# aluo-x/3D_SLN

Measured on AMD Instinct MI355X. Metric: scene-graph VAE steps/sec + 256² diff-render fps, 1/2/4/8 MI355X, higher is better.
Workload: dtype f32; 1 GPU; BASELINE configs[1]: batch=64 scene graphs x (32 objects, 64 triples) per GPU, Sg2ScVAE train step at train.py defaults (embedding_dim=64, 5+5 GraphTripleConv, BatchNorm); O=2048, T=4096, hipgraph=True, distinct_batches_cycled=4, eps=N(0,1) drawn on the device inside the step, parallelism=dp1

## Files before the change

3d_sln_amd/_lib.py:

```python
from __future__ import annotations

import ctypes as C
import os

HERE = os.path.dirname(os.path.abspath(__file__))
LIB_PATH = os.path.join(HERE, "libsln_hip.so")

SLN_E = {-1: "SLN_E_BADARG", -2: "SLN_E_UNSUPPORTED", -3: "SLN_E_STATE", -4: "SLN_E_NOGPU", -5: "SLN_E_NOMEM", -6: "SLN_E_CAPTURE"}

c_f32p = C.c_void_p
c_i64p = C.c_void_p


class SlnError(RuntimeError):
    pass


class SlnVaeConfig(C.Structure):
    _fields_ = [(n, C.c_int) for n in (
        "embedding_dim", "gconv_num_layers", "recurrent", "batch_norm", "decoder_cat", "use_ae",
        "box_dim", "n_angle", "num_objs", "num_preds", "num_attrs", "no_attr")]


class SlnVaeUnit(C.Structure):
# ... 200 lines not shown
                                    C.c_void_p, C.c_int, C.c_int, C.c_int, C.c_void_p, C.c_int64, c_f32p, c_f32p, C.c_void_p]),
    "sln_gconv_net_create": (C.c_int, [C.c_int, C.c_int, C.c_int, C.c_int, C.c_int, C.c_int, C.POINTER(C.c_void_p)]),
    "sln_gconv_net_set_edges": (C.c_int, [C.c_void_p, C.c_void_p, C.c_int, C.c_int, C.c_void_p]),
    "sln_gconv_net_forward": (C.c_int, [C.c_void_p, c_f32p, c_f32p, c_f32p, c_f32p, C.c_int, C.c_void_p]),
    "sln_gconv_net_backward": (C.c_int, [C.c_void_p, c_f32p, c_f32p, c_f32p, c_f32p, C.c_void_p]),
    "sln_linear_forward": (C.c_int, [c_f32p, C.c_int, C.c_int, c_f32p, c_f32p, c_f32p, C.c_int, C.c_void_p,
                                     C.c_int, C.c_void_p]),
    "sln_linear_wgrad": (C.c_int, [c_f32p, c_f32p, C.c_int, C.c_int, C.c_int, c_f32p, c_f32p, C.c_void_p]),
    "sln_debug_gemm_nt": (C.c_int, [C.POINTER(SlnDbgGemmNT), C.c_int, C.POINTER(C.c_int), C.c_void_p]),
    "sln_debug_gemm_tn": (C.c_int, [C.POINTER(SlnDbgGemmTN), C.c_int, C.c_int, C.c_void_p]),
    "sln_debug_gemm_nt_route": (C.c_int, [C.POINTER(SlnDbgGemmNT), C.POINTER(SlnDbgNTRoute)]),
    "sln_debug_gemm_nt_half": (C.c_int, [C.POINTER(SlnDbgGemmNT), C.c_int, C.c_void_p]),
    "sln_debug_gemm_nt_half_takes": (C.c_int, [C.POINTER(SlnDbgGemmNT)]),
    "sln_debug_gemm_sizes": (C.c_int, [C.POINTER(C.c_int), C.c_int]),
    "sln_debug_vae_csr": (C.c_int, [c_i64p, C.c_int, C.c_int, C.c_int, C.POINTER(SlnDbgCsr), C.c_void_p, C.c_void_p]),
    "sln_debug_vae_edge": (C.c_int, [C.POINTER(SlnDbgEdge), C.c_int, C.c_int, C.POINTER(C.c_int), C.c_void_p]),
    "sln_debug_vae_loss": (C.c_int, [C.POINTER(SlnDbgLoss), C.c_void_p]),
    "sln_debug_vae_tables": (C.c_int, [C.c_int, C.c_void_p, C.c_int, C.c_int, C.c_float, C.c_int, C.c_int, C.c_int, C.c_void_p]),
    "sln_debug_vae_embed": (C.c_int, [C.POINTER(SlnDbgEmbed), C.c_int, C.c_int, C.POINTER(C.c_int), C.c_void_p]),
    "sln_debug_vae_opt": (C.c_int, [C.POINTER(SlnDbgOpt), C.c_void_p]),
    "sln_debug_vae_sizes": (C.c_int, [C.POINTER(C.c_int), C.c_int]),
    "sln_debug_vae_leaf_launches": (C.c_int64, [C.c_void_p]),
    "sln_debug_vae_half_launches": (C.c_int64, [C.c_void_p]),
    "sln_project_faces": (C.c_int, [c_f32p, C.c_void_p, c_f32p, c_f32p, c_f32p, C.c_int, C.c_int, C.c_int, C.c_float, C.c_float, c_f32p, C.c_void_p]),
    "sln_project_faces_backward": (C.c_int, [c_f32p, C.c_void_p, c_f32p, c_f32p, c_f32p, C.c_int, C.c_int, C.c_int, C.c_float, C.c_float, c_f32p,
                                             c_f32p, C.c_void_p]),
    "sln_raster_workspace_bytes": (C.c_int64, [C.c_int, C.c_int]),
    "sln_raster_forward": (C.c_int, [c_f32p, C.c_int, C.c_int, C.c_int, C.c_float, C.c_float, C.c_void_p, C.c_void_p,
                                     c_f32p, c_f32p, C.c_void_p]),
    "sln_raster_forward_dual": (C.c_int, [c_f32p, C.c_int, C.c_int, C.c_int, C.c_float, C.c_float, C.c_float, C.c_void_p,
                                          C.c_void_p, c_f32p, c_f32p, C.c_void_p, c_f32p, c_f32p, C.c_void_p]),
    "sln_raster_texture_sample": (C.c_int, [c_f32p, c_f32p, C.c_void_p, c_f32p, c_f32p, C.c_int, C.c_int, C.c_int, C.c_int,
                                            C.c_float, c_f32p, C.c_void_p]),
    "sln_raster_backward_depth": (C.c_int, [c_f32p, C.c_void_p, c_f32p, c_f32p, c_f32p, C.c_int, C.c_int, C.c_int, c_f32p,
                                            C.c_void_p]),
    "sln_raster_backward_rgb": (C.c_int, [c_f32p, C.c_void_p, c_f32p, c_f32p, C.c_int, C.c_int, C.c_int, C.c_int, C.c_float,
                                          c_f32p, C.c_void_p]),
    "sln_raster_texture_sample_chw": (C.c_int, [c_f32p, c_f32p, C.c_void_p, c_f32p, c_f32p, C.c_int, C.c_int, C.c_int, C.c_int, C.c_int,
                                                C.c_float, C.c_float, c_f32p, C.c_void_p]),
    "sln_raster_backward_rgb_multi": (C.c_int, [c_f32p, C.c_void_p, C.c_void_p, C.c_void_p, C.c_int, C.c_int, C.c_int, C.c_int, C.c_float,
                                                C.c_void_p, c_f32p, C.c_void_p]),
    "sln_scene_workspace_bytes": (C.c_int64, [C.c_int, C.c_int, C.c_int]),
    "sln_scene_forward": (C.c_int, [c_f32p, C.c_void_p, C.c_int, C.c_int, C.c_int, C.c_int, C.c_void_p, C.c_void_p,
                                    C.c_float, C.c_float, C.c_float, C.c_float, C.c_void_p, c_f32p, C.c_void_p]),
    "sln_scene_forward_live": (C.c_int, [c_f32p, C.c_void_p, C.c_int, C.c_int, C.c_int, C.c_int, C.c_void_p, C.c_void_p,
                                         C.c_float, C.c_float, C.c_float, C.c_float, C.c_void_p, c_f32p, C.c_void_p, C.c_void_p, C.c_void_p]),
# ... 150 lines not shown
```

3d_sln_amd/csrc/gemm_f32.hip:

```cpp
#include <cstdio>
#include <cstdlib>
#include <algorithm>
#include <vector>
#include "gemm_bodies.h"
#include "vae_multi.h"
namespace {
constexpr bool nt_coef_helpers(int amode, int epi) { return amode != 2 || epi == EPI_MASK; }
template <int BM, int BN, int AMODE, int EPI>
constexpr bool nt_helpers() { return BM == 64 && BN == 64 && nt_coef_helpers(AMODE, EPI); }
template <int BM, int BN, int WM, int WN, int AMODE, int EPI, int MULTI>
__global__ __launch_bounds__((nt_helpers<BM, BN, AMODE, EPI>() ? 512 : 256)) void gemm_nt_kernel(const GemmNTArgs a) {
  extern __shared__ __attribute__((aligned(16))) char smem[];
  gemm_nt_body<BM, BN, WM, WN, AMODE, EPI, MULTI, nt_helpers<BM, BN, AMODE, EPI>()>(a, blockIdx.x, ((a.M + BM - 1) / BM) * ((a.N + BN - 1) / BN), smem);
}

template <int AMODE, int EPI>
constexpr bool nt_helpers2() { return nt_coef_helpers(AMODE, EPI); }
template <int J, int AMODE, int EPI>
__global__ __launch_bounds__((nt_helpers2<AMODE, EPI>() ? 512 : 256)) void gemm_nt16_kernel(const GemmNTArgs a) {
  extern __shared__ __attribute__((aligned(16))) char smem[];
  gemm_nt_body16<J, AMODE, EPI, nt_helpers2<AMODE, EPI>()>(a, blockIdx.x, ((a.M + 63) / 64) * ((a.N + 32 * J - 1) / (32 * J)), smem);
}

template <int AMODE, int EPI, int NSEG = 1>
// ... 264 lines not shown
#define SLN_NT64M(AM, EP, MU) if (am == AM && ep == EP && mu == MU) return launch_nt64_multi<AM, EP, MU>(tab, tiles_dev, R, max_tiles, smem64, st);
    SLN_NT64M(0, EPI_PLAIN, 0) SLN_NT64M(0, EPI_PLAIN, 1) SLN_NT64M(0, EPI_PLAIN, 2) SLN_NT64M(0, EPI_MASK, 0) SLN_NT64M(0, EPI_MASK, 1) SLN_NT64M(0, EPI_MASK, 2)
    SLN_NT64M(2, EPI_PLAIN, 0) SLN_NT64M(2, EPI_PLAIN, 1) SLN_NT64M(2, EPI_PLAIN, 2) SLN_NT64M(2, EPI_MASK, 0) SLN_NT64M(2, EPI_MASK, 1) SLN_NT64M(2, EPI_MASK, 2)
#undef SLN_NT64M
    return -1;
  }
  const size_t smem = nt_small_smem_bytes(max_K);
  const int amode = key / 16, epi = (key / 4) % 4, nseg = key % 4;
#define SLN_NTM(AM, EP, NS) if (amode == AM && epi == EP && nseg == NS) return launch_nt_small_multi<AM, EP, NS>(tab, tiles_dev, R, max_tiles, smem, st);
  SLN_NTM(0, EPI_PLAIN, 1) SLN_NTM(0, EPI_PLAIN, 3) SLN_NTM(0, EPI_MASK, 1) SLN_NTM(0, EPI_MASK, 3)
  SLN_NTM(2, EPI_PLAIN, 1) SLN_NTM(2, EPI_PLAIN, 3) SLN_NTM(2, EPI_MASK, 1) SLN_NTM(2, EPI_MASK, 3)
#undef SLN_NTM
  return -1;
}

int sln_launch_gemm_tn(const GemmTNArgs& a0, hipStream_t st) {
  SlnProfScope prof(SLN_FAM_GEMM_TN, 2.0 * a0.R * a0.Nout * a0.Kin, st);
  GemmTNArgs a = a0;
  const bool x2 = tn_prepare(a);
  if (x2) return launch_tn<64, 64, 2, 2, true>(a, st);
  return launch_tn<64, 64, 2, 2, false>(a, st);
}

int sln_tn_multi_plan(GemmTNArgs* probs, int n, TnMultiMeta* meta, int* blocks, bool* x2, bool* xg, double* flops) {
  if (n < 1 || n > SLN_TN_MULTI_MAX) return -1;
  static const int target0 = std::getenv("SLN_TN_MULTI_ROWS") ? std::atoi(std::getenv("SLN_TN_MULTI_ROWS")) : 768;
  static const bool no_xcd = std::getenv("SLN_TN_NO_XCD") != nullptr;
  bool any_x2 = false, any_xg = false;
  double work = 0.0;
  for (int i = 0; i < n; ++i) {
    const GemmTNArgs& a = probs[i];
    if (a.R <= 0 || a.Nout <= 0 || a.Kin <= 0 || !tn_supported(a)) return -1;
    for (int s = 0; s < a.G.nseg; ++s) any_x2 |= a.G.seg[s].x2 != nullptr;
    any_xg |= tn_gathers(a);
    work += 2.0 * a.R * a.Nout * a.Kin;
  }
  struct Group { int prob, chunk, tiles; long cost; };
  std::vector<Group> groups;
  int per_xcd[8];
  std::vector<int> owner;
  for (long target = g_sln_deterministic ? (1L << 30) : (target0 > 0 ? target0 : 1024);; target *= 2) {
    groups.clear();
    for (int i = 0; i < n; ++i) {
      GemmTNArgs& a = probs[i];
      const int chunks = sln_cdiv(a.R, (int)(target > a.R ? a.R : target));
      a.rows_per_block = sln_cdiv(sln_cdiv(a.R, chunks), BK) * BK;
      const int tiles = sln_cdiv(a.Nout, 64) * sln_cdiv(a.Kin, 64), nch = sln_cdiv(a.R, a.rows_per_block);
      for (int c = 0; c < nch; ++c) {
        const int rows = (c + 1) * a.rows_per_block <= a.R ? a.rows_per_block : a.R - c * a.rows_per_block;
        groups.push_back(Group{i, c, tiles, (long)tiles * rows});
      }
    }
    std::stable_sort(groups.begin(), groups.end(), [](const Group& x, const Group& y) { return x.cost > y.cost; });
    long load[8] = {0, 0, 0, 0, 0, 0, 0, 0};
    for (int x = 0; x < 8; ++x) per_xcd[x] = 0;
    owner.assign(groups.size(), 0);
    for (size_t g = 0; g < groups.size(); ++g) {
      int best = 0;
      if (no_xcd) best = (int)(g % 8);
      else for (int x = 1; x < 8; ++x) if (load[x] < load[best]) best = x;
      owner[g] = best; load[best] += groups[g].cost; per_xcd[best] += groups[g].tiles;
    }
    int mx = 0;
    for (int x = 0; x < 8; ++x) mx = per_xcd[x] > mx ? per_xcd[x] : mx;
    if (8 * mx <= SLN_TN_MULTI_ITEMS) break;
    if (target > (1L << 30)) return -1;
  }
  if (any_xg) {
    const int* any = nullptr;
    for (int i = 0; i < n; ++i) { if (probs[i].X.idx_a) any = probs[i].X.idx_a; else if (probs[i].X.idx_b) any = probs[i].X.idx_b; }
    for (int i = 0; i < n; ++i) if (!probs[i].X.idx_a && !probs[i].X.idx_b) probs[i].X.idx_a = any;
  }
  int mx = 0;
  for (int x = 0; x < 8; ++x) mx = per_xcd[x] > mx ? per_xcd[x] : mx;
  std::memset(meta, 0, sizeof(*meta));
  meta->nprob = n; meta->nblocks = 8 * mx;
  for (int b = 0; b < 8 * mx; ++b) meta->item[b].prob = -1;
  int fill[8] = {0, 0, 0, 0, 0, 0, 0, 0};
  for (size_t g = 0; g < groups.size(); ++g) {
    const int x = owner[g];
    for (int t = 0; t < groups[g].tiles; ++t) {
      TnMultiItem& it = meta->item[8 * (fill[x]++) + x];
      it.prob = groups[g].prob; it.tile = t; it.chunk = groups[g].chunk;
    }
  }
  *blocks = 8 * mx; *x2 = any_x2; *xg = any_xg; *flops = work;
  return 0;
}

int sln_launch_gemm_tn_multi(const GemmTNArgs* dev_probs, const TnMultiMeta* dev_meta, int blocks, bool x2, bool xg, double flops,
                             hipStream_t st) {
  if (blocks <= 0) return 0;
  SlnProfScope prof(SLN_FAM_GEMM_TN, flops, st);
  const size_t smem = tn_smem_bytes(64, 64);
  if (smem > 48 * 1024) { int r = sln_gemm_init(); if (r) return r; }
  if (x2 && xg) hipLaunchKernelGGL((gemm_tn_multi_kernel<true, true>), dim3(blocks), dim3(256), smem, st, dev_probs, dev_meta);
  else if (x2) hipLaunchKernelGGL((gemm_tn_multi_kernel<true, false>), dim3(blocks), dim3(256), smem, st, dev_probs, dev_meta);
  else if (xg) hipLaunchKernelGGL((gemm_tn_multi_kernel<false, true>), dim3(blocks), dim3(256), smem, st, dev_probs, dev_meta);
  else hipLaunchKernelGGL((gemm_tn_multi_kernel<false, false>), dim3(blocks), dim3(256), smem, st, dev_probs, dev_meta);
  SLN_CHECK_LAUNCH();
  return 0;
}

extern "C" int sln_debug_tn_plan(const int* R, const int* Nout, const int* Kin, int n, int* rows_per_block, int* items, int max_items) {
  if (!R || !Nout || !Kin || !rows_per_block || !items || n < 1 || n > SLN_TN_MULTI_MAX) return -1;
  static thread_local GemmTNArgs probs[SLN_TN_MULTI_MAX];
  static thread_local TnMultiMeta meta;
  std::memset(probs, 0, sizeof(GemmTNArgs) * (size_t)n);
  for (int i = 0; i < n; ++i) {
    probs[i].R = R[i]; probs[i].Nout = Nout[i]; probs[i].Kin = Kin[i];
    probs[i].G.nseg = 1; probs[i].X.nseg = 1; probs[i].lddw = i;
  }
  int blocks = 0; bool x2 = false, xg = false; double flops = 0.0;
  const int r = sln_tn_multi_plan(probs, n, &meta, &blocks, &x2, &xg, &flops);
  if (r) return r;
  if (blocks > max_items) return -2;
  for (int i = 0; i < n; ++i) rows_per_block[probs[i].lddw] = probs[i].rows_per_block;
  for (int b = 0; b < blocks; ++b) {
    const TnMultiItem& it = meta.item[b];
    items[3 * b] = it.prob < 0 ? -1 : probs[it.prob].lddw; items[3 * b + 1] = it.tile; items[3 * b + 2] = it.chunk;
  }
  return blocks;
}

#include "sln_debug.h"

bool sln_dbg_bn(const SlnDbgBn& d, int coef, BnView& v) {
  std::memset(&v, 0, sizeof(v));
  v.sums = d.sums; v.gsums = d.gsums; v.gamma = d.gamma; v.beta = d.beta; v.rmean = d.rmean; v.rvar = d.rvar;
  v.cstride = d.cstride; v.mode = d.mode; v.n_rows = d.n_rows; v.eps = d.eps;
  v.rn = 1.0 / (double)(d.n_rows > 0.f ? d.n_rows : 1.f);
  if (coef == SLN_COEF_IDENT || d.mode == SLN_BN_NONE) return d.mode >= SLN_BN_NONE && d.mode <= SLN_BN_EVAL;
  const bool bwd = coef == SLN_COEF_BWD;
  if (d.mode == SLN_BN_TRAIN) return d.gamma && d.sums && d.cstride > 0 && d.n_rows >= 1.f && (bwd ? d.gsums != nullptr : d.beta != nullptr);
  if (d.mode == SLN_BN_EVAL) return d.gamma && d.rvar && (bwd || (d.beta && d.rmean));
  return false;
}
// ... 121 lines not shown
```

3d_sln_amd/csrc/sln_debug.h:

```cpp
#pragma once
#include "sln_common.h"
#include "sln_hip.h"

bool sln_dbg_bn(const SlnDbgBn& d, int coef, BnView& v);
long sln_vae_engine_leaf_launches(const SlnVae* h);
long sln_vae_engine_half_launches(const SlnVae* h);
```

3d_sln_amd/csrc/sln_gemm.h:

```cpp
#pragma once
#include "sln_common.h"

enum { EPI_PLAIN = 0, EPI_STATS = 1, EPI_MASK = 2 };

struct GemmNTArgs {
  Operand A;
  const float* W;
  const float* bias;
  float* Y;
  int ldy, ycol0;
  int M, N, K, ldw;
  const float* addend;
  int ldadd, addcol0;
  double* osums;
  int ocstride;
  int ldx, xcol0;
  const float* xprev;
  double* ogsums;
  BnView obn;
};

struct GemmTNArgs {
  Operand G;
  Operand X;
  float* dW;
  float* db;
  int lddw;
  int R, Nout, Kin;
  int rows_per_block;
  const float* sgd_step;
};

int sln_launch_gemm_nt(const GemmNTArgs& a, int epi, int tile, hipStream_t st);
int sln_launch_gemm_tn(const GemmTNArgs& a, hipStream_t st);
bool sln_nt_half_takes(const GemmNTArgs& a, int epi);
int sln_launch_gemm_nt_half(const GemmNTArgs& a, int terms, hipStream_t st);
int sln_launch_gemm_group(const GemmNTArgs* nt, const int* epi, int n_nt, hipStream_t st);
enum { SLN_TN_MULTI_MAX = 64, SLN_TN_MULTI_ITEMS = 4096 };
struct TnMultiItem { int prob, tile, chunk, pad_; };
struct TnMultiMeta { int nprob, nblocks; TnMultiItem item[SLN_TN_MULTI_ITEMS]; };
int sln_tn_multi_plan(GemmTNArgs* probs, int n, TnMultiMeta* meta, int* blocks, bool* x2, bool* xg, double* flops);
int sln_launch_gemm_tn_multi(const GemmTNArgs* dev_probs, const TnMultiMeta* dev_meta, int blocks, bool x2, bool xg, double flops,
                             hipStream_t st);
int sln_gemm_init();
```

3d_sln_amd/csrc/vae_debug.hip:

```cpp
#include <cstdint>
#include <cstring>
#include <vector>
#include "sln_debug.h"
#include "vae_multi.h"

namespace {

bool dbg_csr(const SlnDbgCsr& d, GraphCsr& g) {
  std::memset(&g, 0, sizeof(g));
  if (d.T < 0 || d.O < 1 || !d.deg || !d.invdeg || !d.rowptr || !d.cursor) return false;
  if (d.T > 0 && (!d.s || !d.p || !d.o || !d.ent)) return false;
  g.s = d.s; g.p = d.p; g.o = d.o; g.deg = d.deg; g.invdeg = d.invdeg; g.rowptr = d.rowptr; g.cursor = d.cursor; g.ent = d.ent;
  g.T = d.T; g.O = d.O;
  return true;
}

bool dbg_fwd_bn(const SlnDbgBn& d, int cols, BnView& v) {
  if (!sln_dbg_bn(d, SLN_COEF_FWD, v)) return false;
  return d.mode != SLN_BN_TRAIN || d.cstride >= cols;
}

enum { E_SCATTER_FWD = 0, E_SCATTER_BWD = 1, E_GATHER_BWD = 2, E_MASK_GSTATS = 3, E_BN_RELU = 4, E_ADD2 = 5 };

bool dbg_edge_ok(const SlnDbgEdge& d, GraphCsr& g, BnView& bn) {
// ... 340 lines not shown
  std::vector<AdamScalars> h(1);
  std::memset(h.data(), 0, sizeof(AdamScalars));
  h[0].step = d->step; h[0].lr = d->lr; h[0].beta1 = d->beta1; h[0].beta2 = d->beta2; h[0].eps = d->eps;
  h[0].rng_seed = d->seed; h[0].rng_offset = d->offset;
  DevTable<AdamScalars> sc;
  int r = sc.upload(h);
  pro.scalars = sc.p;
  for (int k = 0; k < d->calls && !r; ++k)
    r = d->kind == 0   ? sln_launch_adam(d->params, d->grads, d->m, d->v, (long)d->n, sc.p, d->total_loss, st)
        : d->kind == 1 ? sln_launch_randn(d->params, (long)d->n, sc.p, st)
                       : sln_launch_step_prologue(pro, st);
  const int rs = (int)hipStreamSynchronize(st);
  if (!r) r = rs;
  if (!r) r = (int)hipMemcpy(h.data(), sc.p, sizeof(AdamScalars), hipMemcpyDeviceToHost);
  if (sc.p) (void)hipFree(sc.p);
  if (r) return r;
  d->out_step = h[0].step; d->out_offset = h[0].rng_offset; d->out_bc1 = h[0].bc1; d->out_bc2 = h[0].bc2; d->out_skip = h[0].skip;
  if (h[0].adam_done != 0 || h[0].rng_done != 0) return SLN_E_STATE;
  return 0;
}

extern "C" int64_t sln_debug_vae_leaf_launches(const SlnVae* h) { return h ? (int64_t)sln_vae_engine_leaf_launches(h) : (int64_t)SLN_E_BADARG; }
extern "C" int64_t sln_debug_vae_half_launches(const SlnVae* h) { return h ? (int64_t)sln_vae_engine_half_launches(h) : (int64_t)SLN_E_BADARG; }
```

3d_sln_amd/csrc/vae_engine.hip:

```cpp
#include <cstddef>
#include <new>
#include <type_traits>
#include <utility>
#include <vector>
#include <cstring>
#include <cstdlib>

#include "../../include/sln_hip.h"
#include "sln_gemm.h"
#include "vae_kernels.h"
#include "vae_multi.h"
#include "sln_prof.h"

namespace {

enum { SK_DEC_ASSEMBLE = 0, SK_EMBED_GATHER, SK_NT, SK_SCATTER_FWD, SK_TN, SK_TN_FLUSH, SK_MASK_GSTATS, SK_ADD2, SK_EMBED_BWD,
       SK_SCATTER_BWD, SK_GATHER_BWD, SK_DEC_ASSEMBLE_BWD, SK_COPY2D };
struct RecStep {
  int kind = -1, epi = 0, idx64 = 0;
  GemmNTArgs nt; GemmTNArgs tn;
  MScatterFwd sf; MScatterBwd sb; MGatherBwd gb; MMaskGstats mg; MDecAssemble da; DecAssembleBwd dab; MEmbedGather eg; MEmbedBwd eb; MAdd2 a2;
};
struct Recorder { std::vector<RecStep> steps; };

// ... 79 lines not shown
  int dbp_ld = 8;

  bool enc_training = false, dec_training = false, have_enc = false, have_dec = false, have_loss_grads = false;
  const float* z_src = nullptr;
  bool z_from_latent = false;
  bool wt_fresh = false;
  float host_kl = 0.f, host_lr = 0.f; int64_t host_step = 0; bool host_scalars_valid = false;
  float* grad_guard = nullptr;
  bool draw_eps = false;
  unsigned long long host_seed[2] = {0, 0};

  struct TnGroup {
    GemmTNArgs probs[SLN_TN_MULTI_MAX]; TnMultiMeta meta; int n = 0, blocks = 0; bool x2 = false, xg = false; double flops = 0.0;
    bool dirty = true; GemmTNArgs* dev_probs = nullptr; TnMultiMeta* dev_meta = nullptr;
  };
  int tn_slots = 32;
  std::vector<GemmTNArgs> tn_kind_scratch;
  bool capturing = false, tn_upload_pending = false;
  int det_seen = 0;
  bool tn_per_layer = false;
  int tn_slot_next[3] = {0, 0, 0};
  std::vector<GemmTNArgs> deferred;
  TnGroup* tn_groups_store = nullptr;
  TnGroup& tn_group(int set, int slot, int k) { return tn_groups_store[((size_t)set * tn_slots + slot) * 2 + k]; }
  int upload_group(TnGroup& g) {
    hipError_t e = hipMemcpy(g.dev_probs, g.probs, sizeof(GemmTNArgs) * (size_t)g.n, hipMemcpyHostToDevice);
    if (e == hipSuccess) e = hipMemcpy(g.dev_meta, &g.meta, sizeof(TnMultiMeta), hipMemcpyHostToDevice);
    g.dirty = e != hipSuccess;
    return (int)e;
  }
  bool bn_table_live = false;
  struct TnStage { char* host = nullptr; hipEvent_t done = nullptr; };
  enum { TN_STAGE_SLOTS = 16 };
  TnStage tn_stage[TN_STAGE_SLOTS];
  int tn_stage_next = 0;
  int stage_upload(void* dev0, const void* src0, size_t n0, void* dev1, const void* src1, size_t n1, hipStream_t st) {
    hipStreamCaptureStatus cs = hipStreamCaptureStatusNone;
    if (hipStreamIsCapturing(st, &cs) != hipSuccess || cs != hipStreamCaptureStatusNone) return SLN_E_CAPTURE;
    const size_t cap0 = sizeof(GemmTNArgs) * (size_t)SLN_TN_MULTI_MAX, cap = cap0 + sizeof(TnMultiMeta);
    if (n0 > cap0 || n1 > cap - cap0) return SLN_E_BADARG;
    TnStage& sl = tn_stage[tn_stage_next];
    tn_stage_next = (tn_stage_next + 1) % TN_STAGE_SLOTS;
    hipError_t e = hipSuccess;
    if (!sl.host) {
      void* hp = nullptr;
      if (hipHostMalloc(&hp, cap, hipHostMallocDefault) != hipSuccess) return SLN_E_NOMEM;
      sl.host = static_cast<char*>(hp);
      if (hipEventCreateWithFlags(&sl.done, hipEventDisableTiming) != hipSuccess) { (void)hipHostFree(hp); sl.host = nullptr; return SLN_E_NOMEM; }
    } else {
      e = hipEventSynchronize(sl.done);
    }
    if (e == hipSuccess && n0) { std::memcpy(sl.host, src0, n0); e = hipMemcpyAsync(dev0, sl.host, n0, hipMemcpyHostToDevice, st); }
    if (e == hipSuccess && n1) { std::memcpy(sl.host + cap0, src1, n1); e = hipMemcpyAsync(dev1, sl.host + cap0, n1, hipMemcpyHostToDevice, st); }
    if (e == hipSuccess) e = hipEventRecord(sl.done, st);
    return (int)e;
  }
  int upload_group_async(TnGroup& g, hipStream_t st) {
    const int r = stage_upload(g.dev_probs, g.probs, sizeof(GemmTNArgs) * (size_t)g.n, g.dev_meta, &g.meta,
                               offsetof(TnMultiMeta, item) + sizeof(TnMultiItem) * (size_t)g.meta.nblocks, st);
    if (r == 0) g.dirty = false;
    return r;
  }
  int upload_pending_tables() {
    for (int w = 0; w < tn_slots; ++w)
      for (int k = 0; k < 2; ++k) {
        TnGroup& g = tn_group(0, w, k);
        if (g.n > 0 && g.dirty) { int r = upload_group(g); if (r) return r; }
      }
    tn_upload_pending = false;
    return 0;
  }
  hipStream_t tn_eager_stream = nullptr;
  int flush_deferred(int which, hipStream_t st) {
    if (rec) { rec_push(SK_TN_FLUSH); return 0; }
    if (deferred.empty()) return 0;
    const int set = capturing ? 0 : 1;
    if (set == 1 && tn_eager_stream != st) {
      hipStreamCaptureStatus cs = hipStreamCaptureStatusNone, cs_old = hipStreamCaptureStatusNone;
      const bool st_capt = hipStreamIsCapturing(st, &cs) != hipSuccess || cs != hipStreamCaptureStatusNone;
      if (!st_capt) {
        if (tn_eager_stream != nullptr && hipStreamIsCapturing(tn_eager_stream, &cs_old) == hipSuccess && cs_old == hipStreamCaptureStatusNone)
          (void)hipStreamSynchronize(tn_eager_stream);
        tn_eager_stream = st;
      }
    }
    static thread_local TnGroup tmp;
    std::vector<GemmTNArgs>& kind = tn_kind_scratch;
    for (int k = 0; k < 2; ++k) {
      kind.clear();
      for (const GemmTNArgs& t : deferred) {
        bool gathers = false;
        for (int s2 = 0; s2 < t.X.nseg; ++s2) gathers |= t.X.seg[s2].which != 0;
        if ((int)gathers == k) kind.push_back(t);
      }
      size_t next = 0;
      while (next < kind.size()) {
        int want = 0; long tiles = 0;
        for (size_t i = next; i < kind.size() && want < SLN_TN_MULTI_MAX; ++i) {
          const long tl = (long)sln_cdiv(kind[i].Nout, 64) * sln_cdiv(kind[i].Kin, 64);
          if (want > 0 && tiles + tl > SLN_TN_MULTI_ITEMS / 2) break;
          tiles += tl; ++want;
        }
        int r = -1;
        const bool have_slot = tn_slot_next[which] < tn_slots / 3;
        for (; have_slot && want >= 1; want /= 2) {
          tmp.n = want;
          for (int i = 0; i < want; ++i) tmp.probs[i] = kind[next + i];
          r = sln_tn_multi_plan(tmp.probs, tmp.n, &tmp.meta, &tmp.blocks, &tmp.x2, &tmp.xg, &tmp.flops);
          if (r == 0) break;
        }
        if (r != 0) {
          GemmTNArgs one = kind[next++];
          if (g_sln_deterministic) one.rows_per_block = sln_cdiv(one.R, 32) * 32;
          r = sln_launch_gemm_tn(one, st);
          if (r) { deferred.clear(); return r; }
          continue;
        }
        next += (size_t)tmp.n;
        const int slot = which * (tn_slots / 3) + tn_slot_next[which]++;
        TnGroup& g = tn_group(set, slot, k);
        if (g.n != tmp.n || std::memcmp(g.probs, tmp.probs, sizeof(GemmTNArgs) * (size_t)tmp.n) != 0 ||
            std::memcmp(&g.meta, &tmp.meta, sizeof(TnMultiMeta)) != 0) {
          std::memcpy(g.probs, tmp.probs, sizeof(GemmTNArgs) * (size_t)tmp.n);
          g.meta = tmp.meta; g.n = tmp.n; g.blocks = tmp.blocks; g.x2 = tmp.x2; g.xg = tmp.xg; g.flops = tmp.flops;
          g.dirty = true;
        }
        if (g.dirty) {
          if (capturing) tn_upload_pending = true;
          else {
            r = upload_group_async(g, st);
            if (r) { deferred.clear(); return r; }
          }
        }
        r = sln_launch_gemm_tn_multi(g.dev_probs, g.dev_meta, g.blocks, g.x2, g.xg, g.flops, st);
        if (r) { deferred.clear(); return r; }
      }
    }
    deferred.clear();
    return 0;
  }

  hipGraphExec_t graph_exec[4] = {nullptr, nullptr, nullptr, nullptr}; int graph_O[4] = {-1, -1, -1, -1}, graph_T[4] = {-1, -1, -1, -1};

  bool it_zero_in_prologue = false;
  bool it_prologue = false;
  bool it_fused_loss = false;
  bool it_one_flush = false;
  bool one_flush = true;
  bool it_merge_bn = false;
  bool no_merge = false;
  bool it_leaf = false;
  bool it_wt_prologue = false;
  bool leaf_merge = true;
  long leaf_launches = 0;
  int gemm_precision = 0;
  bool in_iteration = false;
  long half_launches = 0;
  bool gconv_only = false;
  int unit_of(int net, int l, int k) const { return (gconv_only ? 0 : 8) + (net * nmod + (cfg.recurrent ? 0 : l)) * 4 + k; }
  int unit_boxnet(int k) const { return 8 + 2 * nmod * 4 + k; }
  int unit_anglenet(int k) const { return 8 + 2 * nmod * 4 + 2 + k; }

  int bn_mode(const BnInst& b, bool training) const {
    if (b.unit < 0 || !units[b.unit].bn) return SLN_BN_NONE;
    return training ? SLN_BN_TRAIN : SLN_BN_EVAL;
  }
  BnView view(int inst, int col0, bool training) const {
    BnView v; std::memset(&v, 0, sizeof(v));
    v.eps = kBnEps; v.n_rows = 1.f; v.rn = 1.0; v.mode = SLN_BN_NONE;
    if (inst < 0) return v;
    const BnInst& b = bns[inst];
// ... 248 lines not shown
  for (auto& ly : layers) {
    const size_t D = ly.Do;
    ly.A1 = b.take<float>(Tm * H); ly.A2 = b.take<float>(Tm * (2 * H + D)); ly.M = b.take<float>(Om * H);
    ly.A3 = b.take<float>(Om * H); ly.A4 = b.take<float>(Om * D);
  }
  hbA1 = b.take<float>(Om * H); hbA2 = b.take<float>(Om * W); haA1 = b.take<float>(Om * H); haA2 = b.take<float>(Om * W);
  mu = b.take<float>(Om * E); logvar = b.take<float>(Om * E); z = b.take<float>(Om * E); eps_buf = b.take<float>(Om * E);
  bnA1 = b.take<float>(Om * H); anA1 = b.take<float>(Om * H);
  boxes_pred = b.take<float>(Om * cfg.box_dim); logits = b.take<float>(Om * cfg.n_angle);
  angles_pred = b.take<float>(Om * cfg.n_angle);
  dbp_ld = rup(cfg.box_dim, 4);
  dbp = b.take<float>(Om * dbp_ld); dlogits = b.take<float>(Om * cfg.n_angle);
  g_bn = b.take<float>(Om * H); g_an = b.take<float>(Om * H);
  d_bx = b.take<float>(Om * (W + n_attr_e)); d_ax = b.take<float>(Om * W);
  const size_t Dm = (size_t)(Dec > Ddc ? Dec : Ddc);
  dM = b.take<float>(Om * H);
  for (auto& ly : layers) {
    const size_t D = ly.Do;
    ly.g4 = b.take<float>(Om * D); ly.g3 = b.take<float>(Om * H); ly.g2 = b.take<float>(Tm * (2 * H + D)); ly.g1 = b.take<float>(Tm * H);
  }
  for (int set = 0; set < 2; ++set)
    for (int w = 0; w < tn_slots; ++w)
      for (int k = 0; k < 2; ++k) {
        GemmTNArgs* dp = b.take<GemmTNArgs>(SLN_TN_MULTI_MAX);
        TnMultiMeta* dm = b.take<TnMultiMeta>(1);
        if (!b.dry && tn_groups_store) {
          TnGroup& tg = tn_group(set, w, k);
          tg.dev_probs = dp; tg.dev_meta = dm; tg.dirty = true; tg.n = 0;
        }
      }
  dG[0] = b.take<float>(Tm * 3 * Dm); dG[1] = b.take<float>(Tm * 3 * Dm);
  dG[2] = (gconv_only || !leaf_merge || no_merge || n_attr_e == 0 || !cfg.decoder_cat) ? nullptr : b.take<float>(Tm * 3 * (size_t)Ddc);
  dX0 = b.take<float>(Om * Dm); dz = b.take<float>(Om * E); dmu = b.take<float>(Om * E); dlv = b.take<float>(Om * E);
  g_h2 = b.take<float>(Om * W); g_h1 = b.take<float>(Om * H); d_xb = b.take<float>(Om * W); d_xa = b.take<float>(Om * W);
  tmp_d = b.take<float>(Om * W);
  g_h2b = b.take<float>(Om * W); g_h1b = b.take<float>(Om * H); tmp_db = b.take<float>(Om * W);
  return (b.off + 255) & ~size_t(255);
}

int SlnVae::refresh_transposes(hipStream_t st) {
  if (wt_fresh) return 0;
  RET_IF(sln_launch_transpose_table(tr_table_dev, n_tr, tr_max_tiles, st));
  wt_fresh = true;
  return 0;
}

VaeLeaf SlnVae::leaf_args() const {
  VaeLeaf v; std::memset(&v, 0, sizeof(v));
// ... 323 lines not shown
    in_iteration = false;
    if (!r) r = loss(boxes_pred, angles_pred, mu, logvar, true, st);
    if (!r && grad_guard && mode != TRAIN_FULL)
      r = (int)hipMemcpyAsync(grad_guard, losses + 3, sizeof(float), hipMemcpyDeviceToDevice, st);
    if (!r) r = decoder_backward(st);
    if (!r) r = sln_launch_latent_bwd(mu, logvar, eps, dz, &scalars->kl_weight, O, E, cfg.use_ae, dmu, dlv, st);
  }
  if (mode != TRAIN_UPTO_DECODER) {
    bulk_zeroed = true;
    if (!r) r = encoder_backward(st);
  }
  bulk_zeroed = false;
  it_prologue = it_fused_loss = it_merge_bn = it_zero_in_prologue = it_one_flush = it_leaf = it_wt_prologue = false;
  RET_IF(r);
  if (mode == TRAIN_FULL) {
    RET_IF(sln_launch_adam(t.flat_params, t.flat_grads, t.adam_m, t.adam_v, (long)t.n_flat, scalars, losses + 3, st));
    wt_fresh = false;
  }
  return 0;
}

long sln_vae_engine_leaf_launches(const SlnVae* h) { return h->leaf_launches; }
long sln_vae_engine_half_launches(const SlnVae* h) { return h->half_launches; }

extern "C" {

int sln_version(void) { return 1; }
const char* sln_build_arch(void) { return "gfx950"; }
int sln_device_ok(void) {
  int n = 0;
  if (hipGetDeviceCount(&n) != hipSuccess || n <= 0) return SLN_E_NOGPU;
  hipDeviceProp_t p;
  int dev = 0;
  if (hipGetDevice(&dev) != hipSuccess || hipGetDeviceProperties(&p, dev) != hipSuccess) return SLN_E_NOGPU;
  return std::strncmp(p.gcnArchName, "gfx950", 6) == 0 ? 0 : SLN_E_NOGPU;
}

static int cfg_check(const SlnVaeConfig* c) {
  if (!c) return SLN_E_BADARG;
  if (c->embedding_dim <= 0 || c->embedding_dim % 16 != 0) return SLN_E_UNSUPPORTED;
  if (c->gconv_num_layers < 1) return SLN_E_UNSUPPORTED;
  if (c->box_dim != 6 && c->box_dim != 4) return SLN_E_UNSUPPORTED;
  if (c->n_angle % 4 != 0 || c->n_angle <= 0) return SLN_E_UNSUPPORTED;
  return 0;
}

int sln_vae_num_units(const SlnVaeConfig* c) {
  if (cfg_check(c) != 0) return cfg_check(c);
  const int nmod = c->recurrent ? 1 : c->gconv_num_layers;
  return 8 + 2 * nmod * 4 + 4;
}

static int read_engine_options(SlnVae* h) {
  auto is = [](const char* name, char c) { const char* v = std::getenv(name); return v && v[0] == c; };
  h->use_group = !is("SLN_NO_GROUP", '1');
  h->no_merge = is("SLN_NO_MERGE", '1');
  h->tn_per_layer = is("SLN_TN_PER_LAYER", '1');
  h->one_flush = !is("SLN_TN_ONE_FLUSH", '0');
  h->leaf_merge = !is("SLN_LEAF_MERGE", '0');
  h->tn_slots = 3 * (2 * h->L + 8 > 16 ? 2 * h->L + 8 : 16);
  h->tn_groups_store = new (std::nothrow) SlnVae::TnGroup[2 * (size_t)h->tn_slots * 2];
  return h->tn_groups_store ? 0 : SLN_E_BADARG;
}

int sln_vae_create(const SlnVaeConfig* c, SlnVae** out) {
  if (!out) return SLN_E_BADARG;
  int r = cfg_check(c);
  if (r != 0) return r;
  SlnVae* h = new (std::nothrow) SlnVae();
  if (!h) return SLN_E_BADARG;
  h->cfg = *c;
  const int E = c->embedding_dim;
  h->E = E; h->H = 4 * E; h->L = c->gconv_num_layers; h->nmod = c->recurrent ? 1 : h->L;
  h->n_obj_e = c->no_attr ? E : E * 3 / 4; h->n_attr_e = c->no_attr ? 0 : E / 4; h->n_box_e = E * 3 / 4; h->n_angle_e = E / 4;
  h->Dec = 2 * E; h->Ddc = c->decoder_cat ? 2 * E : E;
  const int H = h->H, W = 2 * E, n = sln_vae_num_units(c);
  h->units.resize(n);
  auto set = [&](int i, int out_, int in_, bool bn) { h->units[i].out = out_; h->units[i].in = in_; h->units[i].bn = bn && c->batch_norm; };
  set(0, H, W, true); set(1, W, H, true); set(2, h->n_box_e, W, false); set(3, h->n_box_e, W, false);
  set(4, H, W, true); set(5, W, H, true); set(6, h->n_angle_e, W, false); set(7, h->n_angle_e, W, false);
  for (int net = 0; net < 2; ++net)
// ... 556 lines not shown
    if (ev_join) (void)hipEventDestroy(ev_join);
  }
  int fork_side(hipStream_t st) {
    hipError_t e = hipEventRecord(ev_fork, st);
    if (e == hipSuccess) e = hipStreamWaitEvent(side, ev_fork, 0);
    return (int)e;
  }

  int add_single(std::vector<Launch>& prog, const RecStep& st, int room) {
    Launch l; l.kind = L_SINGLE_STEP; l.single = (int)singles.size();
    singles.push_back(st); single_room.push_back(room);
    prog.push_back(l);
    return 0;
  }
  int flush_tn(std::vector<Launch>& prog, std::vector<GemmTNArgs>& pend) {
    static thread_local SlnVae::TnGroup tmp;
    if (!pend.empty()) { Launch f; f.kind = L_FORK; prog.push_back(f); }
    for (int k = 0; k < 2; ++k) {
      std::vector<GemmTNArgs> kind;
      for (const GemmTNArgs& t : pend) if ((int)tn_gathers_host(t) == k) kind.push_back(t);
      size_t next = 0;
      while (next < kind.size()) {
        int want = 0; long tiles = 0;
        for (size_t i = next; i < kind.size() && want < SLN_TN_MULTI_MAX; ++i) {
          const long tl = (long)sln_cdiv(kind[i].Nout, 64) * sln_cdiv(kind[i].Kin, 64);
          if (want > 0 && tiles + tl > SLN_TN_MULTI_ITEMS / 2) break;
          tiles += tl; ++want;
        }
        int r = -1;
        for (; want >= 1; want /= 2) {
          tmp.n = want;
          for (int i = 0; i < want; ++i) tmp.probs[i] = kind[next + i];
          r = sln_tn_multi_plan(tmp.probs, tmp.n, &tmp.meta, &tmp.blocks, &tmp.x2, &tmp.xg, &tmp.flops);
          if (r == 0) break;
        }
        if (r != 0) {
          RecStep st; st.kind = SK_TN; st.tn = kind[next++];
          if (g_sln_deterministic) st.tn.rows_per_block = sln_cdiv(st.tn.R, 32) * 32;
          Launch l; l.kind = L_TN_SINGLE; l.single = (int)singles.size(); l.on_side = true;
          singles.push_back(st); single_room.push_back(-1);
          prog.push_back(l);
          continue;
        }
        next += (size_t)tmp.n;
        Launch l; l.kind = L_TN_MULTI; l.blocks = tmp.blocks; l.x2 = tmp.x2; l.xg = tmp.xg; l.flops = tmp.flops; l.on_side = true;
        std::vector<GemmTNArgs> pv(tmp.probs, tmp.probs + tmp.n);
        RET_IF(upload(pv, &l.tn_probs));
        std::vector<TnMultiMeta> mv(1, tmp.meta);
        RET_IF(upload(mv, &l.tn_meta));
// ... 387 lines not shown
```

include/sln_hip.h:

```cpp
#ifndef SLN_HIP_H
#define SLN_HIP_H

#include <stdint.h>

#ifdef __cplusplus
extern "C" {
#endif

#define SLN_E_BADARG (-1)
#define SLN_E_UNSUPPORTED (-2)
#define SLN_E_STATE (-3)
#define SLN_E_NOGPU (-4)
#define SLN_E_NOMEM (-5)
#define SLN_E_CAPTURE (-6)

int sln_version(void);
const char* sln_build_arch(void);
int sln_device_ok(void);


typedef struct SlnVaeConfig {
  int embedding_dim;
  int gconv_num_layers;
  int recurrent;
// ... 213 lines not shown
  const float* obj_emb; const float* attr_emb; const float* angle_emb; const float* wb; const float* bb;
  const float* mu; const float* logvar; const float* eps; const float* z_in; float* z;
  float* x0; const float* dx0;
  float* d_obj_emb; float* d_attr_emb; float* d_angle_emb; float* d_wb; float* d_bb; float* dz;
  const void* idx; const float* src; void* dst; const float* src2; void* dst2;
  int64_t* st_objs; int64_t* st_attrs; int64_t* st_angles; float* st_boxes; int* attrs32; int* deg; int* err;
  void* zero_ptr; int64_t zero_bytes;
  int kind, O, n_obj, n_attr, n_box, n_angle, box_dim, n_z, use_ae, z_in_x0, rows_obj, rows_attr, rows_angle, ld, col0, n, table_rows,
      T, n2, pad_;
} SlnDbgEmbed;
int sln_debug_vae_embed(const SlnDbgEmbed* desc, int n, int multi, int* variant, void* stream);
typedef struct SlnDbgOpt {
  float* params; const float* grads; float* m; float* v; const float* total_loss; const SlnDbgEmbed* pro;
  int64_t n, step;
  uint64_t seed, offset;
  float lr, beta1, beta2, eps;
  int kind, calls;
  int64_t out_step; uint64_t out_offset; float out_bc1, out_bc2; int out_skip, pad_;
} SlnDbgOpt;
int sln_debug_vae_opt(SlnDbgOpt* desc, void* stream);
int sln_debug_vae_sizes(int* out, int max);
int64_t sln_debug_vae_leaf_launches(const SlnVae* h);
int64_t sln_debug_vae_half_launches(const SlnVae* h);


int sln_project_faces(const float* vertices, const int32_t* faces, const float* K, const float* R, const float* t, int B, int V, int F,
                      float orig_size, float eps, float* faces_xyz, void* stream);
int sln_project_faces_backward(const float* vertices, const int32_t* faces, const float* K, const float* R, const float* t, int B, int V,
                               int F, float orig_size, float eps, const float* grad_faces_xyz, float* grad_vertices, void* stream);
int64_t sln_raster_workspace_bytes(int B, int F);
int sln_raster_forward(const float* faces, int B, int F, int image_size, float near, float far, void* workspace,
                       int32_t* face_index, float* weight, float* depth, void* stream);
int sln_raster_forward_dual(const float* faces, int B, int F, int image_size, float near_a, float near_b, float far,
                            void* workspace, int32_t* fi_a, float* w_a, float* d_a, int32_t* fi_b, float* w_b,
                            float* d_b, void* stream);
int sln_raster_texture_sample(const float* faces, const float* textures, const int32_t* face_index, const float* weight,
                              const float* depth, int B, int F, int image_size, int texture_size, float eps, float* rgb,
                              void* stream);
int sln_raster_backward_depth(const float* faces, const int32_t* face_index, const float* weight, const float* depth,
                              const float* grad_depth, int B, int F, int image_size, float* grad_faces, void* stream);
int sln_raster_backward_rgb(const float* faces, const int32_t* face_index, const float* rgb, const float* grad_rgb, int B,
                            int F, int image_size, int channels, float eps, float* grad_faces, void* stream);
int sln_raster_texture_sample_chw(const float* faces, const float* textures, const int32_t* face_index, const float* weight,
                                  const float* depth, int B, int F, int F_tex, int image_size, int texture_size, float eps, float scale,
                                  float* rgb_chw, void* stream);
int sln_raster_backward_rgb_multi(const float* faces, const int32_t* face_index, const float* const* rgb_chw,
// ... 259 lines not shown
```

Measured before the change: 35360 graphs/s (scene-graph VAE fwd+loss+bwd+Adam).

## Merge all deferred weight-gradient GEMMs into one grouped TN launch

When the single-flush path handles the last deferred batch, every deferred weight-gradient GEMM, both gathering and non-gathering kinds, is planned into one grouped multi-problem launch instead of several per-kind passes. The launch uses a dedicated larger slot with up to 128 problems and 8192 work items. The metadata buffer is sized by item count and the shared index pointer is taken from the largest gathering problem. The aim is fewer kernel launches and graph nodes, plus better XCD load balance in the backward pass. The cost is larger device descriptor buffers and a possible tail imbalance when small and large problems share one grid.

After: 35700 graphs/s (scene-graph VAE fwd+loss+bwd+Adam), median of 6. No clear change (+1.0%).

```diff
diff --git a/3d_sln_amd/_lib.py b/3d_sln_amd/_lib.py
--- a/3d_sln_amd/_lib.py
+++ b/3d_sln_amd/_lib.py
@@ -246,6 +246,7 @@
     "sln_debug_vae_sizes": (C.c_int, [C.POINTER(C.c_int), C.c_int]),
     "sln_debug_vae_leaf_launches": (C.c_int64, [C.c_void_p]),
     "sln_debug_vae_half_launches": (C.c_int64, [C.c_void_p]),
+    "sln_debug_vae_wgrad_launches": (C.c_int64, [C.c_void_p]),
     "sln_project_faces": (C.c_int, [c_f32p, C.c_void_p, c_f32p, c_f32p, c_f32p, C.c_int, C.c_int, C.c_int, C.c_float, C.c_float, c_f32p, C.c_void_p]),
     "sln_project_faces_backward": (C.c_int, [c_f32p, C.c_void_p, c_f32p, c_f32p, c_f32p, C.c_int, C.c_int, C.c_int, C.c_float, C.c_float, c_f32p,
                                              c_f32p, C.c_void_p]),
diff --git a/3d_sln_amd/csrc/gemm_f32.hip b/3d_sln_amd/csrc/gemm_f32.hip
--- a/3d_sln_amd/csrc/gemm_f32.hip
+++ b/3d_sln_amd/csrc/gemm_f32.hip
@@ -310,9 +310,11 @@
   return launch_tn<64, 64, 2, 2, false>(a, st);
 }
 
-int sln_tn_multi_plan(GemmTNArgs* probs, int n, TnMultiMeta* meta, int* blocks, bool* x2, bool* xg, double* flops) {
-  if (n < 1 || n > SLN_TN_MULTI_MAX) return -1;
-  static const int target0 = std::getenv("SLN_TN_MULTI_ROWS") ? std::atoi(std::getenv("SLN_TN_MULTI_ROWS")) : 768;
+int sln_tn_multi_plan(GemmTNArgs* probs, int n, TnMultiMeta* meta, int* blocks, bool* x2, bool* xg, double* flops, int max_items,
+                      bool no_stretch) {
+  if (n < 1 || n > SLN_TN_MULTI_MAX || max_items < 8 || max_items > SLN_TN_MULTI_ITEMS) return -1;
+  static const int rows_env = std::getenv("SLN_TN_MULTI_ROWS") ? std::atoi(std::getenv("SLN_TN_MULTI_ROWS")) : 0;
+  const int target0 = rows_env > 0 ? rows_env : (max_items > SLN_TN_PASS_ITEMS ? 1536 : 768);
   static const bool no_xcd = std::getenv("SLN_TN_NO_XCD") != nullptr;
   bool any_x2 = false, any_xg = false;
   double work = 0.0;
@@ -351,17 +353,25 @@
     }
     int mx = 0;
     for (int x = 0; x < 8; ++x) mx = per_xcd[x] > mx ? per_xcd[x] : mx;
-    if (8 * mx <= SLN_TN_MULTI_ITEMS) break;
+    if (8 * mx <= max_items) break;
+    if (no_stretch) return -1;
     if (target > (1L << 30)) return -1;
   }
   if (any_xg) {
-    const int* any = nullptr;
-    for (int i = 0; i < n; ++i) { if (probs[i].X.idx_a) any = probs[i].X.idx_a; else if (probs[i].X.idx_b) any = probs[i].X.idx_b; }
-    for (int i = 0; i < n; ++i) if (!probs[i].X.idx_a && !probs[i].X.idx_b) probs[i].X.idx_a = any;
+    const int* any = nullptr; int any_rows = 0;
+    for (int i = 0; i < n; ++i) {
+      const int* ip = probs[i].X.idx_a ? probs[i].X.idx_a : probs[i].X.idx_b;
+      if (ip && probs[i].R > any_rows) { any = ip; any_rows = probs[i].R; }
+    }
+    for (int i = 0; i < n; ++i)
+      if (!probs[i].X.idx_a && !probs[i].X.idx_b) {
+        if (probs[i].R > any_rows) return -1;
+        probs[i].X.idx_a = any;
+      }
   }
   int mx = 0;
   for (int x = 0; x < 8; ++x) mx = per_xcd[x] > mx ? per_xcd[x] : mx;
-  std::memset(meta, 0, sizeof(*meta));
+  std::memset(meta, 0, sln_tn_meta_bytes(8 * mx));
   meta->nprob = n; meta->nblocks = 8 * mx;
   for (int b = 0; b < 8 * mx; ++b) meta->item[b].prob = -1;
   int fill[8] = {0, 0, 0, 0, 0, 0, 0, 0};
@@ -400,7 +410,8 @@
     probs[i].G.nseg = 1; probs[i].X.nseg = 1; probs[i].lddw = i;
   }
   int blocks = 0; bool x2 = false, xg = false; double flops = 0.0;
-  const int r = sln_tn_multi_plan(probs, n, &meta, &blocks, &x2, &xg, &flops);
+  const int cap = max_items < SLN_TN_PASS_ITEMS ? SLN_TN_PASS_ITEMS : (max_items > SLN_TN_MULTI_ITEMS ? SLN_TN_MULTI_ITEMS : max_items);
+  const int r = sln_tn_multi_plan(probs, n, &meta, &blocks, &x2, &xg, &flops, cap);
   if (r) return r;
   if (blocks > max_items) return -2;
   for (int i = 0; i < n; ++i) rows_per_block[probs[i].lddw] = probs[i].rows_per_block;
diff --git a/3d_sln_amd/csrc/sln_debug.h b/3d_sln_amd/csrc/sln_debug.h
--- a/3d_sln_amd/csrc/sln_debug.h
+++ b/3d_sln_amd/csrc/sln_debug.h
@@ -5,3 +5,4 @@
 bool sln_dbg_bn(const SlnDbgBn& d, int coef, BnView& v);
 long sln_vae_engine_leaf_launches(const SlnVae* h);
 long sln_vae_engine_half_launches(const SlnVae* h);
+long sln_vae_engine_wgrad_launches(const SlnVae* h);
diff --git a/3d_sln_amd/csrc/sln_gemm.h b/3d_sln_amd/csrc/sln_gemm.h
--- a/3d_sln_amd/csrc/sln_gemm.h
+++ b/3d_sln_amd/csrc/sln_gemm.h
@@ -36,10 +36,13 @@
 bool sln_nt_half_takes(const GemmNTArgs& a, int epi);
 int sln_launch_gemm_nt_half(const GemmNTArgs& a, int terms, hipStream_t st);
 int sln_launch_gemm_group(const GemmNTArgs* nt, const int* epi, int n_nt, hipStream_t st);
-enum { SLN_TN_MULTI_MAX = 64, SLN_TN_MULTI_ITEMS = 4096 };
+enum { SLN_TN_MULTI_MAX = 128, SLN_TN_MULTI_ITEMS = 8192 };
+enum { SLN_TN_PASS_MAX = 64, SLN_TN_PASS_ITEMS = 4096 };
 struct TnMultiItem { int prob, tile, chunk, pad_; };
 struct TnMultiMeta { int nprob, nblocks; TnMultiItem item[SLN_TN_MULTI_ITEMS]; };
-int sln_tn_multi_plan(GemmTNArgs* probs, int n, TnMultiMeta* meta, int* blocks, bool* x2, bool* xg, double* flops);
+int sln_tn_multi_plan(GemmTNArgs* probs, int n, TnMultiMeta* meta, int* blocks, bool* x2, bool* xg, double* flops,
+                      int max_items = SLN_TN_PASS_ITEMS, bool no_stretch = false);
+inline size_t sln_tn_meta_bytes(int items) { return offsetof(TnMultiMeta, item) + sizeof(TnMultiItem) * (size_t)items; }
 int sln_launch_gemm_tn_multi(const GemmTNArgs* dev_probs, const TnMultiMeta* dev_meta, int blocks, bool x2, bool xg, double flops,
                              hipStream_t st);
 int sln_gemm_init();
diff --git a/3d_sln_amd/csrc/vae_debug.hip b/3d_sln_amd/csrc/vae_debug.hip
--- a/3d_sln_amd/csrc/vae_debug.hip
+++ b/3d_sln_amd/csrc/vae_debug.hip
@@ -386,3 +386,4 @@
 
 extern "C" int64_t sln_debug_vae_leaf_launches(const SlnVae* h) { return h ? (int64_t)sln_vae_engine_leaf_launches(h) : (int64_t)SLN_E_BADARG; }
 extern "C" int64_t sln_debug_vae_half_launches(const SlnVae* h) { return h ? (int64_t)sln_vae_engine_half_launches(h) : (int64_t)SLN_E_BADARG; }
+extern "C" int64_t sln_debug_vae_wgrad_launches(const SlnVae* h) { return h ? (int64_t)sln_vae_engine_wgrad_launches(h) : (int64_t)SLN_E_BADARG; }
diff --git a/3d_sln_amd/csrc/vae_engine.hip b/3d_sln_amd/csrc/vae_engine.hip
--- a/3d_sln_amd/csrc/vae_engine.hip
+++ b/3d_sln_amd/csrc/vae_engine.hip
@@ -125,10 +125,13 @@
   int tn_slot_next[3] = {0, 0, 0};
   std::vector<GemmTNArgs> deferred;
   TnGroup* tn_groups_store = nullptr;
+  int tn_big_slot() const { return 2 * (tn_slots / 3); }
+  int tn_slot_probs(int slot) const { return slot == tn_big_slot() ? (int)SLN_TN_MULTI_MAX : (int)SLN_TN_PASS_MAX; }
+  int tn_slot_items(int slot) const { return slot == tn_big_slot() ? (int)SLN_TN_MULTI_ITEMS : (int)SLN_TN_PASS_ITEMS; }
   TnGroup& tn_group(int set, int slot, int k) { return tn_groups_store[((size_t)set * tn_slots + slot) * 2 + k]; }
   int upload_group(TnGroup& g) {
     hipError_t e = hipMemcpy(g.dev_probs, g.probs, sizeof(GemmTNArgs) * (size_t)g.n, hipMemcpyHostToDevice);
-    if (e == hipSuccess) e = hipMemcpy(g.dev_meta, &g.meta, sizeof(TnMultiMeta), hipMemcpyHostToDevice);
+    if (e == hipSuccess) e = hipMemcpy(g.dev_meta, &g.meta, sln_tn_meta_bytes(g.meta.nblocks), hipMemcpyHostToDevice);
     g.dirty = e != hipSuccess;
     return (int)e;
   }
@@ -159,8 +162,7 @@
     return (int)e;
   }
   int upload_group_async(TnGroup& g, hipStream_t st) {
-    const int r = stage_upload(g.dev_probs, g.probs, sizeof(GemmTNArgs) * (size_t)g.n, g.dev_meta, &g.meta,
-                               offsetof(TnMultiMeta, item) + sizeof(TnMultiItem) * (size_t)g.meta.nblocks, st);
+    const int r = stage_upload(g.dev_probs, g.probs, sizeof(GemmTNArgs) * (size_t)g.n, g.dev_meta, &g.meta, sln_tn_meta_bytes(g.meta.nblocks), st);
     if (r == 0) g.dirty = false;
     return r;
   }
@@ -189,19 +191,50 @@
     }
     static thread_local TnGroup tmp;
     std::vector<GemmTNArgs>& kind = tn_kind_scratch;
+    auto gathers_rows = [](const GemmTNArgs& t) {
+      bool gathers = false;
+      for (int s2 = 0; s2 < t.X.nseg; ++s2) gathers |= t.X.seg[s2].which != 0;
+      return gathers;
+    };
+    auto issue = [&](int slot, int k) -> int {
+      TnGroup& g = tn_group(set, slot, k);
+      const size_t mb = sln_tn_meta_bytes(tmp.meta.nblocks);
+      if (g.n != tmp.n || std::memcmp(g.probs, tmp.probs, sizeof(GemmTNArgs) * (size_t)tmp.n) != 0 ||
+          g.meta.nblocks != tmp.meta.nblocks || std::memcmp(&g.meta, &tmp.meta, mb) != 0) {
+        std::memcpy(g.probs, tmp.probs, sizeof(GemmTNArgs) * (size_t)tmp.n);
+        std::memcpy(&g.meta, &tmp.meta, mb); g.n = tmp.n; g.blocks = tmp.blocks; g.x2 = tmp.x2; g.xg = tmp.xg; g.flops = tmp.flops;
+        g.dirty = true;
+      }
+      if (g.dirty) {
+        if (capturing) tn_upload_pending = true;
+        else {
+          const int r = upload_group_async(g, st);
+          if (r) return r;
+        }
+      }
+      ++tn_launches;
+      return sln_launch_gemm_tn_multi(g.dev_probs, g.dev_meta, g.blocks, g.x2, g.xg, g.flops, st);
+    };
+    if (one_launch && it_one_flush && which == 2 && tn_slot_next[2] == 0 && !g_sln_deterministic &&
+        deferred.size() <= (size_t)SLN_TN_MULTI_MAX) {
+      tmp.n = (int)deferred.size();
+      for (int i = 0; i < tmp.n; ++i) tmp.probs[i] = deferred[(size_t)i];
+      if (sln_tn_multi_plan(tmp.probs, tmp.n, &tmp.meta, &tmp.blocks, &tmp.x2, &tmp.xg, &tmp.flops, SLN_TN_MULTI_ITEMS, true) == 0) {
+        const int r = issue(tn_big_slot() + tn_slot_next[2]++, 0);
+        deferred.clear();
+        return r;
+      }
+    }
     for (int k = 0; k < 2; ++k) {
       kind.clear();
-      for (const GemmTNArgs& t : deferred) {
-        bool gathers = false;
-        for (int s2 = 0; s2 < t.X.nseg; ++s2) gathers |= t.X.seg[s2].which != 0;
-        if ((int)gathers == k) kind.push_back(t);
-      }
+      for (const GemmTNArgs& t : deferred)
+        if ((int)gathers_rows(t) == k) kind.push_back(t);
       size_t next = 0;
       while (next < kind.size()) {
         int want = 0; long tiles = 0;
-        for (size_t i = next; i < kind.size() && want < SLN_TN_MULTI_MAX; ++i) {
+        for (size_t i = next; i < kind.size() && want < SLN_TN_PASS_MAX; ++i) {
           const long tl = (long)sln_cdiv(kind[i].Nout, 64) * sln_cdiv(kind[i].Kin, 64);
-          if (want > 0 && tiles + tl > SLN_TN_MULTI_ITEMS / 2) break;
+          if (want > 0 && tiles + tl > SLN_TN_PASS_ITEMS / 2) break;
           tiles += tl; ++want;
         }
         int r = -1;
@@ -215,27 +248,13 @@
         if (r != 0) {
           GemmTNArgs one = kind[next++];
           if (g_sln_deterministic) one.rows_per_block = sln_cdiv(one.R, 32) * 32;
+          ++tn_launches;
           r = sln_launch_gemm_tn(one, st);
           if (r) { deferred.clear(); return r; }
           continue;
         }
         next += (size_t)tmp.n;
-        const int slot = which * (tn_slots / 3) + tn_slot_next[which]++;
-        TnGroup& g = tn_group(set, slot, k);
-        if (g.n != tmp.n || std::memcmp(g.probs, tmp.probs, sizeof(GemmTNArgs) * (size_t)tmp.n) != 0 ||
-            std::memcmp(&g.meta, &tmp.meta, sizeof(TnMultiMeta)) != 0) {
-          std::memcpy(g.probs, tmp.probs, sizeof(GemmTNArgs) * (size_t)tmp.n);
-          g.meta = tmp.meta; g.n = tmp.n; g.blocks = tmp.blocks; g.x2 = tmp.x2; g.xg = tmp.xg; g.flops = tmp.flops;
-          g.dirty = true;
-        }
-        if (g.dirty) {
-          if (capturing) tn_upload_pending = true;
-          else {
-            r = upload_group_async(g, st);
-            if (r) { deferred.clear(); return r; }
-          }
-        }
-        r = sln_launch_gemm_tn_multi(g.dev_probs, g.dev_meta, g.blocks, g.x2, g.xg, g.flops, st);
+        r = issue(which * (tn_slots / 3) + tn_slot_next[which]++, k);
         if (r) { deferred.clear(); return r; }
       }
     }
@@ -250,6 +269,8 @@
   bool it_fused_loss = false;
   bool it_one_flush = false;
   bool one_flush = true;
+  bool one_launch = true;
+  long tn_launches = 0;
   bool it_merge_bn = false;
   bool no_merge = false;
   bool it_leaf = false;
@@ -544,8 +565,8 @@
   for (int set = 0; set < 2; ++set)
     for (int w = 0; w < tn_slots; ++w)
       for (int k = 0; k < 2; ++k) {
-        GemmTNArgs* dp = b.take<GemmTNArgs>(SLN_TN_MULTI_MAX);
-        TnMultiMeta* dm = b.take<TnMultiMeta>(1);
+        GemmTNArgs* dp = b.take<GemmTNArgs>((size_t)tn_slot_probs(w));
+        TnMultiMeta* dm = reinterpret_cast<TnMultiMeta*>(b.take<char>(sln_tn_meta_bytes(tn_slot_items(w))));
         if (!b.dry && tn_groups_store) {
           TnGroup& tg = tn_group(set, w, k);
           tg.dev_probs = dp; tg.dev_meta = dm; tg.dirty = true; tg.n = 0;
@@ -915,6 +936,7 @@
 
 long sln_vae_engine_leaf_launches(const SlnVae* h) { return h->leaf_launches; }
 long sln_vae_engine_half_launches(const SlnVae* h) { return h->half_launches; }
+long sln_vae_engine_wgrad_launches(const SlnVae* h) { return h->tn_launches; }
 
 extern "C" {
 
@@ -950,6 +972,7 @@
   h->no_merge = is("SLN_NO_MERGE", '1');
   h->tn_per_layer = is("SLN_TN_PER_LAYER", '1');
   h->one_flush = !is("SLN_TN_ONE_FLUSH", '0');
+  h->one_launch = !is("SLN_TN_ONE_LAUNCH", '0');
   h->leaf_merge = !is("SLN_LEAF_MERGE", '0');
   h->tn_slots = 3 * (2 * h->L + 8 > 16 ? 2 * h->L + 8 : 16);
   h->tn_groups_store = new (std::nothrow) SlnVae::TnGroup[2 * (size_t)h->tn_slots * 2];
@@ -1552,9 +1575,9 @@
       size_t next = 0;
       while (next < kind.size()) {
         int want = 0; long tiles = 0;
-        for (size_t i = next; i < kind.size() && want < SLN_TN_MULTI_MAX; ++i) {
+        for (size_t i = next; i < kind.size() && want < SLN_TN_PASS_MAX; ++i) {
           const long tl = (long)sln_cdiv(kind[i].Nout, 64) * sln_cdiv(kind[i].Kin, 64);
-          if (want > 0 && tiles + tl > SLN_TN_MULTI_ITEMS / 2) break;
+          if (want > 0 && tiles + tl > SLN_TN_PASS_ITEMS / 2) break;
           tiles += tl; ++want;
         }
         int r = -1;
diff --git a/include/sln_hip.h b/include/sln_hip.h
--- a/include/sln_hip.h
+++ b/include/sln_hip.h
@@ -259,6 +259,7 @@
 int sln_debug_vae_sizes(int* out, int max);
 int64_t sln_debug_vae_leaf_launches(const SlnVae* h);
 int64_t sln_debug_vae_half_launches(const SlnVae* h);
+int64_t sln_debug_vae_wgrad_launches(const SlnVae* h);
 
 
 int sln_project_faces(const float* vertices, const int32_t* faces, const float* K, const float* R, const float* t, int B, int V, int F,
```
